# XingqunQi-lab/EmotionGestures

Hardware: AMD Instinct MI355X
Metric: gesture clips/sec (34 frames, 43 joints) (higher is better)
Workload: dtype bf16x3; 1 GPU; TED clips: 4 s 16 kHz audio -> mel(128x124) -> CVAE sample -> generator -> 34x126 pose; global_batch=64, variant=Models_spatial_memory, parallelism=clip-sharded x1, no data-path collective, launch=hipGraph replay, 4 step(s) in flight, branch_streams=False, fold_affine=False

## Files before the change

emotiongestures_amd/_lib.py:

```python
from __future__ import annotations

import ctypes as C
import os

_HERE = os.path.dirname(os.path.abspath(__file__))
LIB_PATH = os.path.join(_HERE, "libemogest_hip.so")

EG_PREC_F32, EG_PREC_BF16X3, EG_PREC_BF16 = 0, 1, 2
PRECISIONS = {"f32": EG_PREC_F32, "fp32": EG_PREC_F32, "bf16x3": EG_PREC_BF16X3, "bf16": EG_PREC_BF16}

(PACK_RAW, PACK_LINEAR, PACK_VEC_PAD, PACK_CONV3X3, PACK_BN_SCALE, PACK_BN_SHIFT, PACK_CONV1X1, PACK_STEM,
 PACK_WN_TAP, PACK_CONV1D, PACK_POS_TABLE, PACK_LINEAR_T, PACK_LINEAR_FOLD, PACK_BIAS_FOLD, PACK_CONV1X1_BF16, PACK_WN_TAPS) = range(16)


class EgError(RuntimeError):
    pass


class EgWeightEntry(C.Structure):
    _fields_ = [("key", C.c_char * 192), ("kind", C.c_int32), ("dims", C.c_int32 * 4),
                ("offset", C.c_int64), ("numel", C.c_int64)]


class EgGeneratorConfig(C.Structure):
# ... 82 lines not shown
    "eg_resample_stream_reset": (C.c_int, [_P, _I, _I, _I, _P, _P]),
    "eg_resample_stream_push": (C.c_int, [_P, _I, _I, _I, _P, _P, _I, _P, _P, _I, _P]),
    "eg_skeleton_check": (C.c_int, [_P, _P, _P, _I]),
    "eg_skeleton_out_frames": (_L, [_L, _I, _I]),
    "eg_skeleton_tile_frames": (_I, []),
    "eg_skeleton_joints": (C.c_int, [_P, _I, _I, _P, _P, _P, _I, _P, _P, _I, _I, _P, _I, _I, _I, _P, _L, _P]),
    "eg_skeleton_dir_vec": (C.c_int, [_P, _I, _I, _P, _P, _P, _I, _P, _P, _I, _I, _P, _P, _P]),
    "eg_skeleton_rest_check": (C.c_int, [_P, _I]),
    "eg_skeleton_levels": (C.c_int, [_P, _P, _P, _I, _P, _P]),
    "eg_skeleton_rotations": (C.c_int, [_P, _I, _I, _P, _P, _P, _I, _P, _P, _P, _I, _I, _P, _I, _I, _I, _P, _L, _P]),
    "eg_beat_tables": (C.c_int, [_P, _P, _P, _P]),
    "eg_beat_workspace_bytes": (_L, [_I, _I]),
    "eg_beat_align": (C.c_int, [_P, _I, _I, _P, _I, _I, _I, _I, _I, C.c_double, _I, _P, _P, _P, _P, _P, _L, _P, _P, _P, _P, _P, _P, _P]),
    "eg_beat_tracks_meta_ints": (_L, [_I]),
    "eg_beat_tracks_meta": (C.c_int, [_P, _P, _P, _I, _I, _P]),
    "eg_beat_tracks_workspace_bytes": (_L, [_P, _P, _I, _I, _I]),
    "eg_beat_align_tracks": (C.c_int, [_P, _I, _L, _P, _P, _P, _I, _I, _I, _P, _I, _I, _P, C.c_double, _I, _P, _P, _P, _P, _P, _L, _P, _P, _P,
                                       _P, _P, _P, _P]),
    "eg_beat_tracks_scan": (C.c_int, [_P, _P, _I, _P, _P, _L, _P, _P, _P]),
    "eg_take_meta_ints": (_L, [_I]),
    "eg_take_meta": (C.c_int, [_P, _I, _P]),
    "eg_track_rows_pack": (C.c_int, [_P, _I, _I, _I, _I, _P, _P, _P, _P]),
    "eg_take_distance_workspace_bytes": (_L, [_P, _I, _I]),
    "eg_take_distance": (C.c_int, [_P, _I, _I, _I, _P, _P, _I, _P, _L, _P, _P, _P]),
    "eg_conv3x3": (C.c_int, [_P, _P, _P, _P, _P, _P, _P, _I, _I, _I, _I, _I, _I, _I, _I, _I, _P]),
    "eg_conv3x3_se": (C.c_int, [_P, _P, _P, _P, _P, _P, _P, _P, _P, _I, _I, _I, _I, _I, _I, _I, _I, _I, _P]),
    "eg_se_gate_pre": (C.c_int, [_P, _P, _I, _P, _P, _P, _P, _P, _P, _P, _P, _I, _I, _I, _I, _P]),
    "eg_se_block_fused": (C.c_int, [_P] * 19 + [_I] * 7 + [_P]),
    "eg_conv3x3_gap_tiles": (_I, [_I, _I, _I, _I, _I]),
    "eg_conv3x3_channel_split": (_I, [_I, _I, _I, _I, _I, _I, _I]),
    "eg_stem_conv": (C.c_int, [_P, _P, _P, _P, _P, _P, _I, _I, _I, _I, _P]),
    "eg_se_gate": (C.c_int, [_P, _I, _P, _P, _P, _P, _P, _I, _I, _I, _P]),
    "eg_se_residual_relu": (C.c_int, [_P, _P, _P, _P, _P, _P, _P, _I, _I, _I, _I, _I, _I, _I, _I, _P]),
    "eg_linear": (C.c_int, [_P, _I, _P, _I, _P, _P, _P, _I, _P, _I, _I, _I, _I, _I, _I, _I, _I, _P]),
    "eg_split_tiles": (C.c_int, [_P, _I, _I, _I, _P, _P]),
    "eg_linear_presplit": (C.c_int, [_P, _I, _P, _I, _P, _P, _P, _I, _P, _I, _I, _I, _I, _I, _I, _P]),
    "eg_linear_presplit_causal": (C.c_int, [_P, _I, _P, _P, _I, _P, _P, _I, _P, _I, _P, _I, _I, _I, _I, _I, _I, _I, _I, _P]),
    "eg_linear_splitk": (C.c_int, [_P, _I, _P, _I, _P, _P, _I, _I, _I, _I, _I, _I, _P, _I, _P]),
    "eg_layernorm": (C.c_int, [_P, _P, _P, _P, _I, _I, C.c_float, _P]),
    "eg_attention": (C.c_int, [_P, _I, _P, _I, _P, _I, _P, _I, _P, _I, _I, _I, _I, _I, _I, _P]),
    "eg_attention_masked": (C.c_int, [_P, _I, _P, _I, _P, _I, _P, _L, _I, _P, _I, _P, _I, _I, _I, _I, _I, _I, _P]),
    "eg_mha_workspace_bytes": (_L, [_I, _I, _I, _I, _I]),
    "eg_multi_head_attention": (C.c_int, [_P, _P, _P, _P, _P, _P, _P, _P, _P, _P, _I, _I, _I, _I, _I, _I, _P, _L, _P]),
    "eg_ffn_workspace_bytes": (_L, [_I, _I, _I]),
    "eg_positionwise_ffn": (C.c_int, [_P, _P, _P, _P, _P, _P, _P, _P, _I, _I, _I, _I, _P, _L, _P]),
    "eg_tcn_forward": (C.c_int, [_P, _P, _P, _I, _I, _I, _I, _I, _P, _L, _P]),
    "eg_add_rows": (C.c_int, [_P, _P, _P, _L, _I, _I, _P]),
    "eg_add_rows_split": (C.c_int, [_P, _P, _P, _P, _L, _I, _I, _P]),
    "eg_conv3x3_packed_floats": (_L, [_I, _I]),
    "eg_profile_enable": (C.c_int, [_I]),
    "eg_profile_disable": (C.c_int, []),
    "eg_profile_read": (_I, [_P, _P, _P, _I]),
    "eg_profile_read_workgroups": (_I, [_P, _I]),
    "eg_reparameterize": (C.c_int, [_P, _P, _P, _P, _L, _P]),
    "eg_conv1d": (C.c_int, [_P, _P, _P, _P, _P, _P, _I, _I, _I, _I, _I, _I, _I, _I, _P]),
    "eg_contrastive_workspace_bytes": (C.c_int64, [_I]),
    "eg_contrastive_loss": (C.c_int, [_P, _P, _I, _I, _P, _P, _P, _P, _L, _P]),
    "eg_contrastive_backward_workspace_bytes": (_L, [_I]),
    "eg_contrastive_loss_backward": (C.c_int, [_P, _P, _I, _I, _P, _P, _P, _L, _P]),
    "eg_transpose": (C.c_int, [_P, _I, _I, _I, _P, _I, _P]),
    "eg_gemm_tn_workspace_floats": (_L, [_I, _I, _L]),
    "eg_gemm_tn": (C.c_int, [_P, _I, _P, _I, _P, _I, _I, _I, _L, _P, _L, _I, _P]),
    "eg_conv3x3_wgrad": (C.c_int, [_P, _P, _P, _I, _I, _I, _I, _I, _I, _P, _L, _P]),
    "eg_im2col3x3": (C.c_int, [_P, _P, _I, _I, _I, _I, _I, _I, _P]),
    "eg_subsample": (C.c_int, [_P, _P, _I, _I, _I, _I, _I, _I, _P]),
    "eg_conv1d_cl_forward": (C.c_int, [_P, _P, _P, _P] + [_I] * 9 + [_P]),
    "eg_conv1d_cl_backward_input": (C.c_int, [_P, _P, _P, _P] + [_I] * 9 + [_P]),
    "eg_conv1d_cl_backward_weight_workspace_floats": (_L, [_I] * 7),
    "eg_conv1d_cl_backward_weight": (C.c_int, [_P, _P, _P, _P, _P] + [_I] * 9 + [_P, _L, _P]),
    "eg_pad_cols": (C.c_int, [_P, _P, _L, _I, _I, _P]),
    "eg_colreduce_workspace_floats": (_L, [_I]),
    "eg_bn_train_forward": (C.c_int, [_P, _P, _P, _P, _P, _P, _P, _P, _L, _I, C.c_float, C.c_float, _P, _P]),
    "eg_bn_train_backward": (C.c_int, [_P, _P, _P, _P, _P, _P, _P, _P, _L, _I, _I, _P, _P]),
    "eg_bn_train_forward_gap": (C.c_int, [_P, _P, _I, _I, _P, _P, _P, _P, _P, _P, _P, _P, _L, _I, C.c_float, C.c_float, _P, _P]),
    "eg_bn_train_forward_sq": (C.c_int, [_P, _P, _P, _I, _I, _P, _P, _P, _P, _P, _P, _P, _P, _L, _I, C.c_float, C.c_float, _P, _P]),
    "eg_conv3x3_sq": (C.c_int, [_P, _P, _P, _P, _P, _P] + [_I] * 8 + [_P]),
    "eg_se_gate_train_forward": (C.c_int, [_P] * 12 + [_I, _I, _I, _P]),
    "eg_se_tail_forward": (C.c_int, [_P] * 9 + [_I, _I, _I, _P]),
    "eg_se_tail_backward_reduce": (C.c_int, [_P] * 7 + [_I, _I, _I, _P, _P]),
    "eg_se_gate_train_backward": (C.c_int, [_P] * 16 + [_I, _I, _I, _P]),
    "eg_se_tail_backward_finish": (C.c_int, [_P] * 14 + [_I, _I, _I, _P]),
    "eg_se_tail_backward_apply": (C.c_int, [_P] * 13 + [_I, _I, _I, _P]),
    "eg_colsum": (C.c_int, [_P, _P, _P, _P, _L, _I, _P, _P]),
    "eg_elementwise": (C.c_int, [_P, _P, _P, _L, _I, C.c_float, _P]),
    "eg_conv3x3_wgrad_mfma_workspace_floats": (_L, [_I, _I, _I, _I, _I]),
    "eg_conv3x3_wgrad_mfma": (C.c_int, [_P, _P, _P, _I, _I, _I, _I, _I, _P, _L, _P]),
    "eg_conv3x3_wgrad_mfma_oihw": (C.c_int, [_P, _P, _P, _I, _I, _I, _I, _I, _P, _L, _P]),
    "eg_conv3x3_wgrad_gather_mfma": (C.c_int, [_P, _P, _P, _I, _I, _I, _I, _I, _I, _P, _L, _P]),
    "eg_conv3x3_dgrad_s2": (C.c_int, [_P, _P, _P, _P, _I, _I, _I, _I, _I, _I, _P]),
    "eg_conv3x3_res_masked": (C.c_int, [_P, _P, _P, _P, _P, _I, _I, _I, _I, _I, _I, _P]),
    "eg_conv3x3_wgrad_mfma_oihw_in_affine": (C.c_int, [_P, _P, _P, _P, _P, _I, _I, _I, _I, _I, _P, _L, _P]),
    "eg_conv3x3_sq_in_affine": (C.c_int, [_P, _P, _P, _P, _P, _P, _P, _P, _I, _I, _I, _I, _I, _I, _I, _I, _P]),
    "eg_bn_train_stats_sq": (C.c_int, [_P, _P, _I, _I, _P, _P, _P, _P, _P, _P, _P, _P, _L, _I, C.c_float, C.c_float, _P, _P]),
    "eg_pack_conv3x3_device": (C.c_int, [_P, _I, _I, _I, _P, _P]),
    "eg_linear_packed_floats": (_L, [_I, _I]),
    "eg_pack_linear_device": (C.c_int, [_P, _I, _I, _I, _I, _P, _P]),
    "eg_pack_table_blocks": (_I, [_I, _I, _I, _I]),
    "eg_pack_table": (C.c_int, [_P, _I, _I, _P]),
    "eg_dropout": (C.c_int, [_P, _P, _L, C.c_float, C.c_uint32, C.c_uint64, _P]),
    "eg_dropout_dev": (C.c_int, [_P, _P, _L, C.c_float, C.c_uint32, C.c_uint64, _P, _P]),
    "eg_seg_mean": (C.c_int, [_P, _P, _I, _I, _I, C.c_float, _P, _P]),
    "eg_seg_dot": (C.c_int, [_P, _P, _P, _I, _I, _I, _P, _P]),
    "eg_se_scale": (C.c_int, [_P, _P, _P, _P, _I, _I, _I, _P]),
    "eg_layernorm_backward": (C.c_int, [_P, _P, _P, _P, _P, _I, _I, C.c_float, _P]),
    "eg_attention_train": (C.c_int, [_P, _I, _P, _I, _P, _I, _P, _I, _P, _I, _I, _I, _I, _I, C.c_float, C.c_uint32, C.c_uint64, _P, _P]),
    "eg_attention_backward_train": (C.c_int, [_P, _I, _P, _I, _P, _I, _P, _P, _I, _P, _I, _P, _I, _P, _I, _I, _I, _I, _I, _I, C.c_float, C.c_uint32,
# ... 57 lines not shown
```

emotiongestures_amd/csrc/mel.hip:

```cpp
#include "common.h"
#include "beat_shared.h"
#include <hip/hip_fp16.h>
#include <math.h>

namespace {

__global__ __launch_bounds__(256) void mel_power_kernel(const float* __restrict__ audio, int n_samples, const float* __restrict__ melfb_t,
                                                        const float* __restrict__ window, const float* __restrict__ twiddle,
                                                        const int* __restrict__ band, float* __restrict__ melpow, int n_frames) {
    __shared__ float re[1024], im[1024];
    const int f0 = blockIdx.x * 2, f1 = f0 + 1, b = blockIdx.y, tid = threadIdx.x;
    const float* clip = audio + (size_t)b * n_samples;
    for (int i = tid; i < 1024; i += 256) {
        const int s0 = f0 * 512 - 512 + i, s1 = s0 + 512;
        const float wv = window[i];
        const int r = (int)(__brev((unsigned)i) >> 22);
        re[r] = (s0 >= 0 && s0 < n_samples) ? clip[s0] * wv : 0.f;
        im[r] = (f1 < n_frames && s1 >= 0 && s1 < n_samples) ? clip[s1] * wv : 0.f;
    }
    __syncthreads();
#pragma unroll 1
    for (int s = 0; s < 10; ++s) {
        const int half = 1 << s;
#pragma unroll
        for (int u = 0; u < 2; ++u) {
            const int j = tid + u * 256;
            const int pos = j & (half - 1), i0 = ((j >> s) << (s + 1)) + pos, i1 = i0 + half;
            const int tw = pos << (9 - s);
            const float c = twiddle[2 * tw], sn = twiddle[2 * tw + 1];
            const float xr = re[i1], xi = im[i1];
            const float tr = xr * c - xi * sn, ti = xr * sn + xi * c;
            const float ar = re[i0], ai = im[i0];
            re[i0] = ar + tr; im[i0] = ai + ti;
            re[i1] = ar - tr; im[i1] = ai - ti;
        }
        __syncthreads();
    }
    float pa[3], pb[3];
#pragma unroll
    for (int u = 0; u < 3; ++u) {
        const int k = u < 2 ? tid + u * 256 : 512, nk = (1024 - k) & 1023;
        pa[u] = pb[u] = 0.f;
        if (u < 2 || tid == 0) {
            const float zr = re[k], zi = im[k], yr = re[nk], yi = im[nk];
            const float r0 = 0.5f * (zr + yr), i0 = 0.5f * (zi - yi);
            const float r1 = 0.5f * (zi + yi), i1 = 0.5f * (yr - zr);
            pa[u] = r0 * r0 + i0 * i0;
            pb[u] = r1 * r1 + i1 * i1;
        }
    }
    __syncthreads();
    re[tid] = pa[0]; re[tid + 256] = pa[1];
    im[tid] = pb[0]; im[tid + 256] = pb[1];
    if (tid == 0) { re[512] = pa[2]; im[512] = pb[2]; }
    __syncthreads();
    const int m = tid & 127, fr = tid >> 7, f = f0 + fr;
    const float* pw = fr ? im : re;
    const int b0 = band[2 * m], b1 = band[2 * m + 1];
    float s = 0.f;
    for (int k = b0; k < b1; ++k) s += melfb_t[k * 128 + m] * pw[k];
    if (f < n_frames) melpow[((size_t)b * 128 + m) * n_frames + f] = s;
}

__global__ __launch_bounds__(1024) void mel_db_kernel(const float* __restrict__ melpow, float* __restrict__ spec, int n_frames,
                                                      int out_frames) {
    __shared__ float red[16];
    const int b = blockIdx.x, tid = threadIdx.x;
    const float* p = melpow + (size_t)b * 128 * n_frames;
    float mx = 0.f;
    for (int i = tid; i < 128 * n_frames; i += 1024) mx = fmaxf(mx, p[i]);
    mx = wave_max(mx);
    if ((tid & 63) == 0) red[tid >> 6] = mx;
    __syncthreads();
    mx = red[0];
#pragma unroll
    for (int w = 1; w < 16; ++w) mx = fmaxf(mx, red[w]);
    const float inv_ref = 1.0f / fmaxf(1e-10f, mx);
    const float floor_db = -80.f;
    for (int i = tid; i < 128 * out_frames; i += 1024) {
        const int m = i / out_frames, f = i - m * out_frames;
        float db = 10.f * log10f(fmaxf(1e-10f, p[m * n_frames + f]) * inv_ref);
        db = fmaxf(db, floor_db);
        spec[((size_t)b * 128 + m) * out_frames + f] = __half2float(__float2half_rn(db));
    }
}

double hz_to_mel(double f) {
    const double f_sp = 200.0 / 3, min_log_hz = 1000.0, min_log_mel = min_log_hz / f_sp, logstep = log(6.4) / 27.0;
    return f >= min_log_hz ? min_log_mel + log(f / min_log_hz) / logstep : f / f_sp;
}
double mel_to_hz(double m) {
    const double f_sp = 200.0 / 3, min_log_hz = 1000.0, min_log_mel = min_log_hz / f_sp, logstep = log(6.4) / 27.0;
    return m >= min_log_mel ? min_log_hz * exp(logstep * (m - min_log_mel)) : f_sp * m;
}

}

namespace {

void mel_tables_host(int n_fft, float* h_melfb_t, float* h_window, float* h_twiddle, int32_t* h_band) {
    const int n_mels = 128, n_bins = n_fft / 2 + 1;
    const double sr = 16000.0;
    double hz[130];
    const double m_lo = hz_to_mel(0.0), m_hi = hz_to_mel(sr / 2);
    for (int i = 0; i < n_mels + 2; ++i) hz[i] = mel_to_hz(m_lo + (m_hi - m_lo) * i / (n_mels + 1));
    for (int m = 0; m < n_mels; ++m) {
        const double enorm = 2.0 / (hz[m + 2] - hz[m]);
        for (int k = 0; k < n_bins; ++k) {
            const double fk = (sr / 2) * k / (n_bins - 1);
            const double lower = (fk - hz[m]) / (hz[m + 1] - hz[m]);
            const double upper = (hz[m + 2] - fk) / (hz[m + 2] - hz[m + 1]);
            double w = lower < upper ? lower : upper;
            if (w < 0) w = 0;
            h_melfb_t[k * 128 + m] = (float)(w * enorm);
        }
        int lo = n_bins, hi = 0;
        for (int k = 0; k < n_bins; ++k)
            if (h_melfb_t[k * 128 + m] != 0.f) { if (k < lo) lo = k; hi = k + 1; }
        if (lo > hi) lo = hi = 0;
        h_band[2 * m] = lo; h_band[2 * m + 1] = hi;
    }
    const double pi = 3.14159265358979323846;
    for (int i = 0; i < n_fft; ++i) h_window[i] = (float)(0.5 - 0.5 * cos(2.0 * pi * i / n_fft));
    for (int t = 0; t < n_fft / 2; ++t) {
        h_twiddle[2 * t] = (float)cos(2.0 * pi * t / n_fft);
        h_twiddle[2 * t + 1] = (float)(-sin(2.0 * pi * t / n_fft));
    }
}

}

extern "C" int eg_mel_tables(float* h_melfb_t, float* h_window, float* h_twiddle, int32_t* h_band) {
    EG_REQUIRE(h_melfb_t && h_window && h_twiddle && h_band, EG_ERR_BAD_ARG, "eg_mel_tables: null pointer");
    mel_tables_host(1024, h_melfb_t, h_window, h_twiddle, h_band);
    return EG_OK;
}

extern "C" int64_t eg_mel_workspace_bytes(int32_t batch, int32_t n_samples) {
    const int n_frames = 1 + n_samples / 512;
    return (int64_t)batch * 128 * n_frames * (int64_t)sizeof(float);
}

extern "C" int eg_melspectrogram(const float* audio, int32_t batch, int32_t n_samples, const float* d_melfb_t,
                                 const float* d_window, const float* d_twiddle, const int32_t* d_band, float* spec, int32_t out_frames,
                                 void* workspace, int64_t workspace_bytes, void* stream) {
    EG_REQUIRE(audio && d_melfb_t && d_window && d_twiddle && d_band && spec && workspace, EG_ERR_BAD_ARG, "eg_melspectrogram: null pointer");
    EG_REQUIRE(batch > 0 && n_samples >= 512, EG_ERR_BAD_ARG, "eg_melspectrogram: batch=%d n_samples=%d", batch, n_samples);
    const int n_frames = 1 + n_samples / 512;
    EG_REQUIRE(out_frames > 0 && out_frames <= n_frames, EG_ERR_BAD_ARG, "eg_melspectrogram: out_frames=%d of %d", out_frames, n_frames);
    EG_REQUIRE(workspace_bytes >= eg_mel_workspace_bytes(batch, n_samples), EG_ERR_WORKSPACE, "eg_melspectrogram: workspace too small");
    hipStream_t st = (hipStream_t)stream;
    float* melpow = reinterpret_cast<float*>(workspace);
    hipLaunchKernelGGL(mel_power_kernel, dim3((n_frames + 1) / 2, batch), dim3(256), 0, st, audio, n_samples, d_melfb_t, d_window, d_twiddle,
                       d_band, melpow, n_frames);
    int rc = eg_check_launch("mel_power");
    if (rc) return rc;
    hipLaunchKernelGGL(mel_db_kernel, dim3(batch), dim3(1024), 0, st, melpow, spec, n_frames, out_frames);
    return eg_check_launch("mel_db");
}

#define EG_BEAT_MAX_EVENTS (EG_BEAT_MAX_FRAMES / 2 + 1)

namespace {

__global__ __launch_bounds__(256) void beat_stft_kernel(const float* __restrict__ audio, int n_samples, const float* __restrict__ melfb_t,
                                                        const float* __restrict__ window, const float* __restrict__ twiddle,
                                                        const int* __restrict__ band, float* __restrict__ meldb, float* __restrict__ rms,
                                                        int n_frames) {
    const int b = blockIdx.y;
    beat_stft_frames(audio + (size_t)b * n_samples, n_samples, melfb_t, window, twiddle, band, meldb + (size_t)b * 128 * n_frames,
                     rms + (size_t)b * n_frames, n_frames, blockIdx.x * 2);
}

__device__ double gahr(const short* __restrict__ ev, int n_ev, const short* __restrict__ pb, int n_pb, int fps, double sigma) {
    return beat_gahr(ev, n_ev, pb, n_pb, fps, sigma);
}

__global__ __launch_bounds__(256) void beat_align_kernel(const float* __restrict__ meldb, const float* __restrict__ rms_ws, int n_frames,
                                                         const float* __restrict__ pose, int pose_frames, int pose_dim, int fps, int r_lo,
                                                         int r_hi, double sigma, int order, double* __restrict__ score,
                                                         int* __restrict__ n_audio_beats, float* __restrict__ oenv_out,
                                                         float* __restrict__ rms_out, uint8_t* __restrict__ audio_mask,
                                                         uint8_t* __restrict__ pose_mask) {
    __shared__ float oenv[EG_BEAT_MAX_FRAMES], x[EG_BEAT_MAX_FRAMES], rms[EG_BEAT_MAX_FRAMES];
    __shared__ uint8_t fl[3][EG_BEAT_MAX_FRAMES];
    uint8_t* cand = fl[0];
    uint8_t* min_o = fl[1];
    uint8_t* min_r = fl[2];
    __shared__ short ev[3][EG_BEAT_MAX_EVENTS];
    __shared__ float vel[8][EG_BEAT_MAX_FRAMES];
    __shared__ short pbeat[8][EG_BEAT_MAX_EVENTS];
    __shared__ int n_pb[8];
    __shared__ float redf[2][4];
    __shared__ int n_ev_s, any_s;
    __shared__ double g24[24];
    const int b = blockIdx.x, tid = threadIdx.x, T = n_frames;
    const float* db = meldb + (size_t)b * 128 * T;

    float mx = -INFINITY;
    for (int i = tid; i < 128 * T; i += 256) mx = fmaxf(mx, db[i]);
    mx = wave_max(mx);
    if ((tid & 63) == 0) redf[0][tid >> 6] = mx;
    __syncthreads();
    const float floor_db = fmaxf(fmaxf(redf[0][0], redf[0][1]), fmaxf(redf[0][2], redf[0][3])) - 80.f;
    for (int t = tid; t < T; t += 256) {
        float s = 0.f;
        if (t >= 3)
// ... 173 lines not shown
```

emotiongestures_amd/csrc/misc.hip:

```cpp
#include "common.h"

namespace {

template <int NV>
__global__ __launch_bounds__(256) void layernorm_kernel(const float* __restrict__ x, const float* __restrict__ g,
                                                        const float* __restrict__ b, float* __restrict__ y, int rows, int D,
                                                        float eps, unsigned short* __restrict__ img) {
    const int row = blockIdx.x * 4 + (threadIdx.x >> 6), lane = threadIdx.x & 63;
    if (row >= rows) return;
    const f4* xr = reinterpret_cast<const f4*>(x + (size_t)row * D);
    const int nq = D >> 2;
    f4 v[NV];
    float s = 0.f;
#pragma unroll
    for (int i = 0; i < NV; ++i) {
        const int q = lane + i * 64;
        v[i] = q < nq ? xr[q] : (f4){0.f, 0.f, 0.f, 0.f};
        s += (v[i][0] + v[i][1]) + (v[i][2] + v[i][3]);
    }
    const float m0 = wave_sum(s) / (float)D;
    float c = 0.f;
#pragma unroll
    for (int i = 0; i < NV; ++i) {
        const int q = lane + i * 64;
        if (q < nq) {
            const f4 d = v[i] - m0;
            c += (d[0] + d[1]) + (d[2] + d[3]);
        }
    }
    const float mean = m0 + wave_sum(c) / (float)D;
    float ss = 0.f;
#pragma unroll
    for (int i = 0; i < NV; ++i) {
        const int q = lane + i * 64;
        if (q < nq) {
            const f4 d = v[i] - mean;
            ss += (d[0] * d[0] + d[1] * d[1]) + (d[2] * d[2] + d[3] * d[3]);
        }
    }
    const float rstd = 1.0f / sqrtf(wave_sum(ss) / (float)D + eps);
    f4* yr = reinterpret_cast<f4*>(y + (size_t)row * D);
#pragma unroll
    for (int i = 0; i < NV; ++i) {
        const int q = lane + i * 64;
        if (q < nq) {
            const f4 o = (v[i] - mean) * rstd * reinterpret_cast<const f4*>(g)[q] + reinterpret_cast<const f4*>(b)[q];
            yr[q] = o;
            if (img) {
                const f4 z = (f4){0.f, 0.f, 0.f, 0.f};
                bf8 h8, l8;
                split_octet<true>(o, z, h8, l8);
                const int KO = D >> 3;
                const size_t slot = (((size_t)(row >> 6) * KO + (q >> 1)) * 64 + (row & 63)) * 8 + (q & 1) * 4;
// ... 51 lines not shown
    const size_t total = (size_t)((rows + 63) >> 6) * 64 * KO;
    for (size_t i = (size_t)blockIdx.x * 256 + threadIdx.x; i < total; i += (size_t)gridDim.x * 256) {
        if (zero && i < (size_t)64 * KO) zero[i] = (bf8){0, 0, 0, 0, 0, 0, 0, 0};
        const int t = (int)(i / (64 * KO)), rem = (int)(i - (size_t)t * 64 * KO), o = rem >> 6, r = t * 64 + (rem & 63), k = o * 8;
        if (r >= rows) continue;
        int64_t w = idx[r];
        w = w < 0 ? 0 : (w >= n_words ? n_words - 1 : w);
        f4 v0 = (f4){0.f, 0.f, 0.f, 0.f}, v1 = v0;
        if (k < dim) v0 = *reinterpret_cast<const f4*>(table + (size_t)w * dim + k);
        if (k + 4 < dim) v1 = *reinterpret_cast<const f4*>(table + (size_t)w * dim + k + 4);
        *reinterpret_cast<f4*>(out + (size_t)r * ld + k) = v0;
        *reinterpret_cast<f4*>(out + (size_t)r * ld + k + 4) = v1;
        bf8 h, l;
        split_octet<true>(v0, v1, h, l);
        const size_t slot = ((size_t)(r >> 6) * KO + o) * 64 + (r & 63);
        hi[slot] = h;
        lo[slot] = l;
    }
}

__global__ __launch_bounds__(256) void add_kernel(const f4* __restrict__ a, const f4* __restrict__ b, f4* __restrict__ out,
                                                  size_t n4, int row_q, int period) {
    for (size_t i = (size_t)blockIdx.x * 256 + threadIdx.x; i < n4; i += (size_t)gridDim.x * 256) {
        size_t j = i;
        if (period) {
            const size_t row = i / row_q;
            j = (row % period) * row_q + (i - row * row_q);
        }
        out[i] = a[i] + b[j];
    }
}

__global__ __launch_bounds__(256) void add_img_kernel(const f4* __restrict__ a, const f4* __restrict__ b, f4* __restrict__ out, bf8* __restrict__ hi,
                                                      bf8* __restrict__ lo, size_t rows, int row_o, int period) {
    const size_t total = ((rows + 63) >> 6) * 64 * row_o;
    for (size_t t = (size_t)blockIdx.x * 256 + threadIdx.x; t < total; t += (size_t)gridDim.x * 256) {
        const size_t tile = t / (64 * (size_t)row_o);
        const int rem = (int)(t - tile * 64 * row_o), o = rem >> 6;
        const size_t row = tile * 64 + (rem & 63);
        if (row >= rows) continue;
        const size_t i = row * row_o + o;
        const size_t j = period ? (row % period) * row_o + o : i;
        const f4 v0 = a[2 * i] + b[2 * j], v1 = a[2 * i + 1] + b[2 * j + 1];
        out[2 * i] = v0;
        out[2 * i + 1] = v1;
        bf8 h, l;
        split_octet<true>(v0, v1, h, l);
        const size_t slot = ((row >> 6) * row_o + o) * 64 + (row & 63);
        hi[slot] = h;
        lo[slot] = l;
    }
}

__global__ __launch_bounds__(256) void time_linear_kernel(const float* __restrict__ x, const float* __restrict__ w,
                                                          const float* __restrict__ bias, float* __restrict__ y, int L, int C, int ld) {
    extern __shared__ __attribute__((aligned(16))) float sm[];
    float* Ws = sm;
    float* Xs = sm + L * L;
    const int b = blockIdx.y, c0 = blockIdx.x * 64, tid = threadIdx.x;
    for (int i = tid; i < L * L; i += 256) Ws[i] = w[i];
    for (int i = tid; i < L * 64; i += 256) {
        const int t = i >> 6, c = i & 63;
        Xs[i] = (c0 + c < C) ? x[((size_t)b * L + t) * ld + c0 + c] : 0.f;
    }
    __syncthreads();
    const int c = tid & 63;
    if (c0 + c >= C) return;
    for (int tp = tid >> 6; tp < L; tp += 4) {
        float s = bias[tp];
        for (int t = 0; t < L; ++t) s += Ws[tp * L + t] * Xs[t * 64 + c];
        y[((size_t)b * L + tp) * ld + c0 + c] = s;
    }
}

struct PriorArgs {
    const float* prior;
    const float *w1, *b1, *s1, *t1;
    const float *w2, *b2, *s2, *t2;
    const float *sp_w0, *sp_b0, *sp_w1, *sp_b1;
    const float *tc_w0, *tc_b0, *tc_w1, *tc_b1;
    const float *tm_w0, *tm_b0, *tm_w1, *tm_b1;
    float* cat;
    float* tm_mem;
    float* tm_pe;
    int P, PL, D, Dpad, chunk, variant, stage_w, dchunk;
};

__device__ __forceinline__ float block_dot(const float* __restrict__ wrow, const float* __restrict__ xs, int n, int lane) {
    float s = 0.f;
    for (int i = lane; i < n; i += 64) s += wrow[i] * xs[i];
    return wave_sum(s);
}

__global__ __launch_bounds__(256) void prior_pred_kernel(PriorArgs a) {
    extern __shared__ __attribute__((aligned(16))) float sm[];
    const int b = blockIdx.x, tid = threadIdx.x, wave = tid >> 6, lane = tid & 63;
    const int P = a.P, PL = a.PL, D = a.D;
    const int d0 = blockIdx.y * a.dchunk, dc = min(a.dchunk, D - d0);
    const int XW = dc + 4, HW = dc + 2;
    float* xs = sm;
    float* h1 = xs + P * XW;
    float* h2 = h1 + PL * HW;
    float* v0 = h2 + PL * dc;
    float* v1 = v0 + (a.variant == 1 ? a.chunk * D : 0);
    float* v2 = v1 + (a.variant == 1 ? D : 0);
    float* w1s = v2 + (a.variant == 1 ? D : 0);
    float* w2s = w1s + PL * P * 3;
    if (a.stage_w) {
        for (int i = tid; i < PL * P * 3; i += 256) w1s[i] = a.w1[i];
        for (int i = tid; i < PL * PL * 3; i += 256) w2s[i] = a.w2[i];
    }
    const float* w1p = a.stage_w ? w1s : a.w1;
    const float* w2p = a.stage_w ? w2s : a.w2;
    for (int i = tid; i < P * XW; i += 256) {
        const int f = i / XW, d = d0 - 2 + (i - f * XW);
        xs[i] = (d >= 0 && d < D) ? a.prior[((size_t)b * P + f) * D + d] : 0.f;
    }
    __syncthreads();
    for (int i = tid; i < PL * HW; i += 256) {
        const int co = i / HW, j = i - co * HW, d = d0 - 1 + j;
        float v = 0.f;
        if (d >= 0 && d < D) {
            float s = a.b1[co];
            for (int ci = 0; ci < P; ++ci) {
                const float* wp = w1p + (co * P + ci) * 3;
// ... 529 lines not shown
    EG_REQUIRE(a && table && out && images && rows > 0 && d > 0 && (d & 63) == 0, EG_ERR_BAD_ARG, "eg_add_rows_split: null pointer, empty shape or d %% 64 != 0");
    return egi_add_img(a, table, out, images, (size_t)rows * d, d, period, (hipStream_t)stream);
}

extern "C" int eg_window_gather(const float* audio, int32_t utterances, int64_t total_samples, int32_t windows, int64_t hop_samples,
                                int32_t n_samples, float* out, void* stream) {
    EG_REQUIRE(audio && out, EG_ERR_BAD_ARG, "eg_window_gather: null pointer");
    EG_REQUIRE(utterances >= 1 && windows >= 1, EG_ERR_BAD_ARG, "eg_window_gather: utterances=%d windows=%d", utterances, windows);
    EG_REQUIRE(total_samples >= 1 && hop_samples >= 1 && n_samples >= 1, EG_ERR_BAD_ARG, "eg_window_gather: total_samples=%lld hop_samples=%lld n_samples=%d",
               (long long)total_samples, (long long)hop_samples, n_samples);
    EG_REQUIRE((int64_t)(windows - 1) * hop_samples < total_samples, EG_ERR_BAD_ARG,
               "eg_window_gather: windows=%d: the last window starts at sample %lld of %lld", windows, (long long)(windows - 1) * hop_samples,
               (long long)total_samples);
    hipLaunchKernelGGL(window_gather_kernel, dim3(grid_for((size_t)utterances * windows * n_samples)), dim3(256), 0, (hipStream_t)stream, audio, out,
                       utterances, total_samples, windows, hop_samples, n_samples);
    return eg_check_launch("window_gather");
}

int egi_embedding(const int64_t* idx, const float* table, float* out, int rows, int dim, int ld, int n_words, hipStream_t st) {
    hipLaunchKernelGGL(embedding_kernel, dim3(grid_for((size_t)rows * dim / 4)), dim3(256), 0, st, idx, table, out, rows, dim, ld, n_words);
    return eg_check_launch("embedding");
}
int egi_add(const float* a, const float* b, float* out, size_t n, int row_len, int period, hipStream_t st);
int egi_embedding_img(const int64_t* idx, const float* table, float* out, void* img, void* zero_line, int rows, int dim, int ld, int n_words, hipStream_t st) {
    EG_REQUIRE((dim & 3) == 0 && (ld & 63) == 0 && ld >= dim, EG_ERR_ALIGN, "embedding: dim %% 4, ld %% 64");
    bf8* hi = reinterpret_cast<bf8*>(img);
    bf8* lo = hi + (size_t)eg_cdiv(rows, 64) * (ld >> 3) * 64;
    hipLaunchKernelGGL(embedding_img_kernel, dim3(grid_for((size_t)eg_cdiv(rows, 64) * 64 * (ld >> 3))), dim3(256), 0, st, idx, table, out, hi, lo,
                       reinterpret_cast<bf8*>(zero_line), rows, dim, ld, n_words);
    return eg_check_launch("embedding");
}
int egi_add_img(const float* a, const float* b, float* out, void* img, size_t n, int row_len, int period, hipStream_t st) {
    if (!img) return egi_add(a, b, out, n, row_len, period, st);
    EG_REQUIRE((row_len & 63) == 0, EG_ERR_ALIGN, "add: image output needs row_len %% 64 == 0");
    const size_t rows = n / row_len;
    bf8* hi = reinterpret_cast<bf8*>(img);
    bf8* lo = hi + ((rows + 63) >> 6) * (size_t)(row_len >> 3) * 64;
    hipLaunchKernelGGL(add_img_kernel, dim3(grid_for(n / 8)), dim3(256), 0, st, reinterpret_cast<const f4*>(a), reinterpret_cast<const f4*>(b),
                       reinterpret_cast<f4*>(out), hi, lo, rows, row_len / 8, period);
    return eg_check_launch("add");
}
int egi_add(const float* a, const float* b, float* out, size_t n, int row_len, int period, hipStream_t st) {
    hipLaunchKernelGGL(add_kernel, dim3(grid_for(n / 4)), dim3(256), 0, st, reinterpret_cast<const f4*>(a),
                       reinterpret_cast<const f4*>(b), reinterpret_cast<f4*>(out), n / 4, row_len / 4, period);
    return eg_check_launch("add");
}
int egi_add_bcast(const float* a, const float* b, float* out, size_t rows, int row_len, int period, int rep, hipStream_t st) {
    const size_t n4 = rows * (size_t)(row_len / 4);
    hipLaunchKernelGGL(add_bcast_kernel, dim3(grid_for(n4)), dim3(256), 0, st, reinterpret_cast<const f4*>(a),
                       reinterpret_cast<const f4*>(b), reinterpret_cast<f4*>(out), n4, row_len / 4, period, rep);
    return eg_check_launch("add_bcast");
}
int egi_time_linear(const float* x, const float* w, const float* bias, float* y, int batch, int L, int C, int ld, hipStream_t st) {
    const size_t smem = sizeof(float) * ((size_t)L * L + (size_t)L * 64);
    hipLaunchKernelGGL(time_linear_kernel, dim3(eg_cdiv(C, 64), batch), dim3(256), smem, st, x, w, bias, y, L, C, ld);
    return eg_check_launch("time_linear");
}
int egi_copy2d(const float* src, int lds_, float* dst, int ldd, int rows, int cols, hipStream_t st) {
    hipLaunchKernelGGL(copy2d_kernel, dim3(grid_for((size_t)rows * cols)), dim3(256), 0, st, src, lds_, dst, ldd, rows, cols);
    return eg_check_launch("copy2d");
}

int egi_swap01(const void* in, void* out, int A, int B, size_t inner_words, hipStream_t st) {
    if ((inner_words & 3) == 0 && eg_aligned16(in) && eg_aligned16(out)) {
        const size_t q = inner_words / 4;
        hipLaunchKernelGGL((swap01_kernel<u32x4_t>), dim3(grid_for((size_t)A * B * q)), dim3(256), 0, st, reinterpret_cast<const u32x4_t*>(in),
                           reinterpret_cast<u32x4_t*>(out), A, B, q);
    } else {
        hipLaunchKernelGGL((swap01_kernel<unsigned int>), dim3(grid_for((size_t)A * B * inner_words)), dim3(256), 0, st,
                           reinterpret_cast<const unsigned int*>(in), reinterpret_cast<unsigned int*>(out), A, B, inner_words);
    }
    return eg_check_launch("swap01");
}
int egi_rollout_handoff(const float* pose, const float* prior_in, const float* alpha, float* track, float* windows, float* prior_out, int U,
                        int W, int w, int F, int P, int D, hipStream_t st) {
    hipLaunchKernelGGL(rollout_handoff_kernel, dim3(grid_for((size_t)U * F * D)), dim3(256), 0, st, pose, prior_in, alpha, track, windows,
                       prior_out, U, W, w, F, P, D);
    return eg_check_launch("rollout_handoff");
}

struct EgiPriorW {
    const float *w1, *b1, *s1, *t1, *w2, *b2, *s2, *t2;
    const float *sp_w0, *sp_b0, *sp_w1, *sp_b1, *tc_w0, *tc_b0, *tc_w1, *tc_b1, *tm_w0, *tm_b0, *tm_w1, *tm_b1;
};
int egi_prior_encoder(const float* prior, const EgiPriorW& w, float* cat, float* tm_mem, float* tm_pe, float* tm_gram,
                      int batch, int P, int F, int D, int Dpad, int chunk, int variant, hipStream_t st) {
    PriorArgs a;
    a.prior = prior; a.w1 = w.w1; a.b1 = w.b1; a.s1 = w.s1; a.t1 = w.t1; a.w2 = w.w2; a.b2 = w.b2; a.s2 = w.s2; a.t2 = w.t2;
    a.sp_w0 = w.sp_w0; a.sp_b0 = w.sp_b0; a.sp_w1 = w.sp_w1; a.sp_b1 = w.sp_b1;
    a.tc_w0 = w.tc_w0; a.tc_b0 = w.tc_b0; a.tc_w1 = w.tc_w1; a.tc_b1 = w.tc_b1;
    a.tm_w0 = w.tm_w0; a.tm_b0 = w.tm_b0; a.tm_w1 = w.tm_w1; a.tm_b1 = w.tm_b1;
    a.cat = cat; a.tm_mem = tm_mem; a.tm_pe = tm_pe;
    a.P = P; a.PL = F - P; a.D = D; a.Dpad = Dpad; a.chunk = chunk; a.variant = variant;
    const int PL = F - P;
    a.dchunk = variant == 1 ? D : (D < 64 ? D : 64);
    const int dc = a.dchunk;
    const size_t base = sizeof(float) * ((size_t)P * (dc + 4) + (size_t)PL * (dc + 2) + (size_t)PL * dc +
                                         (variant == 1 ? (size_t)chunk * D + 2 * (size_t)D : 0));
    const size_t wbytes = sizeof(float) * ((size_t)PL * P * 3 + (size_t)PL * PL * 3);
    a.stage_w = (base + wbytes <= 160 * 1024) ? 1 : 0;
    const size_t smem = base + (a.stage_w ? wbytes : 0);
    if (smem > 160 * 1024) { eg_set_error("prior encoder: LDS need %zu B", smem); return EG_ERR_UNSUPPORTED; }
    if (int rc = eg_ensure_dynamic_lds(reinterpret_cast<const void*>(prior_pred_kernel), smem, "prior encoder")) return rc;
    hipLaunchKernelGGL(prior_pred_kernel, dim3(batch, eg_cdiv(D, dc)), dim3(256), smem, st, a);
    int rc = eg_check_launch("prior_pred");
    if (rc || variant != 1) return rc;
    hipLaunchKernelGGL(tm_gram_kernel, dim3(eg_cdiv(D * chunk, 256)), dim3(256), 0, st, tm_mem, tm_pe, tm_gram, batch, D, chunk);
    if ((rc = eg_check_launch("tm_gram"))) return rc;
    hipLaunchKernelGGL(tm_apply_kernel, dim3(batch), dim3(64), 0, st, tm_mem, tm_gram, cat, D, Dpad, chunk, P, F);
// ... 275 lines not shown
```

include/emogest.h:

```cpp
#ifndef EMOGEST_H
#define EMOGEST_H

#include <stddef.h>
#include <stdint.h>

#ifdef __cplusplus
extern "C" {
#endif

typedef enum EgStatus {
    EG_OK = 0,
    EG_ERR_BAD_ARG = -1,
    EG_ERR_UNSUPPORTED = -2,
    EG_ERR_WORKSPACE = -3,
    EG_ERR_HIP = -4,
    EG_ERR_ALIGN = -5
} EgStatus;

typedef enum EgPrecision {
    EG_PREC_F32 = 0,
    EG_PREC_BF16X3 = 1,
    EG_PREC_BF16 = 2
} EgPrecision;

// ... 273 lines not shown
                       int32_t m, int32_t n, int32_t k, int32_t relu, int32_t precision, void* stream);
int eg_linear_presplit_causal(const void* x_images, int32_t k_x, const void* zero_line, const float* w, int32_t ldw, const float* bias,
                              const float* res2, int32_t ldr, float* y, int32_t ldc, void* y_images, int32_t y_k, int32_t m, int32_t n,
                              int32_t k_tap, int32_t relu, int32_t shift, int32_t period, int32_t precision, void* stream);

int eg_linear_splitk(const float* x, int32_t lda, const float* w, int32_t ldw, const float* bias, float* y,
                     int32_t ldc, int32_t m, int32_t n, int32_t k, int32_t relu, int32_t splits,
                     float* partial, int32_t precision, void* stream);

typedef struct EgLinearArgs {
    const float* x; const float* w; const float* bias; const float* res1; const float* res2; float* y;
    const float* gate_src;
    const int32_t* drop_epoch;
    float* partial;
    const void* x_images;
    void* y_images;
    uint64_t drop_offset;
    int32_t lda, ldw, ldr, ldc, ldg;
    int32_t m, n, k, relu, precision, splits;
    int32_t k_x, y_k;
    uint32_t drop_seed;
    float drop_p;
} EgLinearArgs;
int eg_linear_ex(const EgLinearArgs* args, void* stream);

int eg_layernorm(const float* x, const float* gamma, const float* beta, float* y, int32_t rows, int32_t d,
                 float eps, void* stream);
int eg_layernorm_img(const float* x, const float* gamma, const float* beta, float* y, void* y_images, int32_t rows, int32_t d, float eps,
                     void* stream);

int eg_attention(const float* q, int32_t ldq, const float* k, int32_t ldk, const float* v, int32_t ldv,
                 float* out, int32_t ldo, float* attn, int32_t batch, int32_t heads, int32_t lq, int32_t lk,
                 int32_t dk, int32_t precision, void* stream);
int eg_attention_masked(const float* q, int32_t ldq, const float* k, int32_t ldk, const float* v, int32_t ldv, const uint8_t* mask,
                        int64_t mask_batch_stride, int32_t mask_query_stride, float* out, int32_t ldo, float* attn, int32_t batch,
                        int32_t heads, int32_t lq, int32_t lk, int32_t dk, int32_t precision, void* stream);

int64_t eg_mha_workspace_bytes(int32_t batch, int32_t lq, int32_t lk, int32_t d_model, int32_t heads);
int eg_multi_head_attention(const float* xq, const float* xkv, const float* wq, const float* wk, const float* wv,
                            const float* wo, const float* ln_g, const float* ln_b, float* out, float* attn,
                            int32_t batch, int32_t lq, int32_t lk, int32_t d_model, int32_t heads,
                            int32_t precision, void* workspace, int64_t workspace_bytes, void* stream);

int64_t eg_ffn_workspace_bytes(int32_t rows, int32_t d_model, int32_t d_inner);
int eg_positionwise_ffn(const float* x, const float* w1, const float* b1, const float* w2, const float* b2,
                        const float* ln_g, const float* ln_b, float* out, int32_t rows, int32_t d_model,
                        int32_t d_inner, int32_t precision, void* workspace, int64_t workspace_bytes, void* stream);

int eg_tcn_forward(const float* x, const float* w, float* y, int32_t batch, int32_t len, int32_t c,
                   int32_t levels, int32_t precision, void* workspace, int64_t workspace_bytes, void* stream);

int eg_add_rows_split(const float* a, const float* table, float* out, void* images, int64_t rows, int32_t d, int32_t period, void* stream);
int eg_add_rows(const float* a, const float* table, float* out, int64_t rows, int32_t d, int32_t period, void* stream);

int eg_reparameterize(const float* mu, const float* logvar, const float* eps, float* z, int64_t n, void* stream);

int eg_conv1d(const float* x, const float* w, const float* bias, const float* scale, const float* shift, float* y, int32_t n,
              int32_t cin, int32_t cout, int32_t lin, int32_t k, int32_t stride, int32_t pad, int32_t act, void* stream);

int64_t eg_contrastive_workspace_bytes(int32_t n);
int eg_contrastive_loss(const float* face, const float* audio, int32_t n, int32_t d, float* cross, float* loss, float* acc,
                        void* workspace, int64_t workspace_bytes, void* stream);
int64_t eg_contrastive_backward_workspace_bytes(int32_t n);
int eg_contrastive_loss_backward(const float* face, const float* audio, int32_t n, int32_t d, float* gface, float* gaudio, void* workspace,
                                 int64_t workspace_bytes, void* stream);



int eg_transpose(const float* x, int32_t ldx, int32_t rows, int32_t cols, float* y, int32_t ldy, void* stream);
int64_t eg_gemm_tn_workspace_floats(int32_t m, int32_t n, int64_t k);
int eg_gemm_tn(const float* a, int32_t lda, const float* b, int32_t ldb, float* c, int32_t ldc, int32_t m, int32_t n, int64_t k,
               float* workspace, int64_t workspace_floats, int32_t accumulate, void* stream);
int eg_conv3x3_wgrad(const float* x, const float* dy, float* dw_mat, int32_t batch, int32_t h, int32_t w, int32_t cin, int32_t cout,
                     int32_t stride, float* workspace, int64_t workspace_floats, void* stream);
int eg_im2col3x3(const float* x, float* col, int32_t batch, int32_t h, int32_t w, int32_t c, int32_t stride, int32_t backward, void* stream);
int eg_subsample(const float* x, float* y, int32_t batch, int32_t h, int32_t w, int32_t c, int32_t stride, int32_t backward, void* stream);
int eg_conv1d_cl_forward(const float* x, const float* w, const float* bias, float* y, int32_t batch, int32_t len, int32_t cin, int32_t len_out,
                         int32_t cout, int32_t k, int32_t stride, int32_t pad, int32_t dilation, void* stream);
int eg_conv1d_cl_backward_input(const float* dy, const float* w, const float* bias, float* dx, int32_t batch, int32_t len, int32_t cin,
                                int32_t len_out, int32_t cout, int32_t k, int32_t stride, int32_t pad, int32_t dilation, void* stream);
int64_t eg_conv1d_cl_backward_weight_workspace_floats(int32_t batch, int32_t cin, int32_t len_out, int32_t cout, int32_t k, int32_t stride,
                                                      int32_t dilation);
int eg_conv1d_cl_backward_weight(const float* x, const float* dy, float* dw, float* db_dy, float* db_x, int32_t batch, int32_t len, int32_t cin,
                                 int32_t len_out, int32_t cout, int32_t k, int32_t stride, int32_t pad, int32_t dilation, float* workspace,
                                 int64_t workspace_floats, void* stream);
int eg_pad_cols(const float* x, float* y, int64_t rows, int32_t k, int32_t k_padded, void* stream);
int64_t eg_colreduce_workspace_floats(int32_t c);
int eg_bn_train_forward(const float* x, const float* gamma, const float* beta, float* y, float* save_mean, float* save_rstd,
                        float* running_mean, float* running_var, int64_t rows, int32_t c, float momentum, float eps, float* workspace,
                        void* stream);
int eg_bn_train_backward(const float* x, const float* dy, const float* gamma, const float* save_mean, const float* save_rstd, float* dx,
                         float* dgamma, float* dbeta, int64_t rows, int32_t c, int32_t relu_mask, float* workspace, void* stream);
int eg_bn_train_forward_gap(const float* x, const float* gap_partial, int32_t tiles, int32_t batch, const float* gamma, const float* beta,
                            float* y, float* save_mean, float* save_rstd, float* clip_sum, float* running_mean, float* running_var,
                            int64_t rows, int32_t c, float momentum, float eps, float* workspace, void* stream);
int eg_bn_train_forward_sq(const float* x, const float* gap_partial, const float* gap_sq_partial, int32_t tiles, int32_t batch, const float* gamma,
                           const float* beta, float* y, float* save_mean, float* save_rstd, float* clip_sum, float* running_mean, float* running_var,
                           int64_t rows, int32_t c, float momentum, float eps, float* workspace, void* stream);
int eg_bn_train_stats_sq(const float* gap_partial, const float* gap_sq_partial, int32_t tiles, int32_t batch, const float* gamma, const float* beta,
                         float* save_mean, float* save_rstd, float* running_mean, float* running_var, float* aff_scale, float* aff_shift, int64_t rows,
                         int32_t c, float momentum, float eps, float* workspace, void* stream);
int eg_se_gate_train_forward(const float* clip_sum, const float* mean, const float* rstd, const float* gamma, const float* beta, const float* w1,
                             const float* b1, const float* w2, const float* b2, float* pooled, float* h, float* gate, int32_t batch, int32_t hw,
                             int32_t c, void* stream);
int eg_se_tail_forward(const float* c2, const float* res, const float* mean, const float* rstd, const float* gamma, const float* beta,
                       const float* gate, float* out, uint32_t* relu_bits, int32_t batch, int32_t hw, int32_t c, void* stream);
// ... 74 lines not shown
```

Baseline: 27040 clips/s.

## Use radix-4 mel FFT and register-blocked time-linear kernel

Replaces the radix-2 shared-memory FFT in the mel power kernel with a five-pass radix-4 FFT. It keeps values in registers between passes, uses swizzled LDS slots and twiddles staged in LDS, and unrolls the mel filterbank dot product by eight. Rewrites the time-linear kernel so each thread accumulates several output rows in registers, reading padded weights as float4 and staging loads in batches. The old kernels stay selectable through environment variables, and a public eg_time_linear entry point is added. The extra getenv calls add host cost per launch, though hipGraph replay hides that.

```diff
diff --git a/emotiongestures_amd/_lib.py b/emotiongestures_amd/_lib.py
--- a/emotiongestures_amd/_lib.py
+++ b/emotiongestures_amd/_lib.py
@@ -158,6 +158,7 @@
     "eg_profile_disable": (C.c_int, []),
     "eg_profile_read": (_I, [_P, _P, _P, _I]),
     "eg_profile_read_workgroups": (_I, [_P, _I]),
+    "eg_time_linear": (C.c_int, [_P, _P, _P, _P, _I, _I, _I, _I, _P]),
     "eg_reparameterize": (C.c_int, [_P, _P, _P, _P, _L, _P]),
     "eg_conv1d": (C.c_int, [_P, _P, _P, _P, _P, _P, _I, _I, _I, _I, _I, _I, _I, _I, _P]),
     "eg_contrastive_workspace_bytes": (C.c_int64, [_I]),
diff --git a/emotiongestures_amd/csrc/mel.hip b/emotiongestures_amd/csrc/mel.hip
--- a/emotiongestures_amd/csrc/mel.hip
+++ b/emotiongestures_amd/csrc/mel.hip
@@ -2,12 +2,14 @@
 #include "beat_shared.h"
 #include <hip/hip_fp16.h>
 #include <math.h>
+#include <stdlib.h>
+#include <string.h>
 
 namespace {
 
-__global__ __launch_bounds__(256) void mel_power_kernel(const float* __restrict__ audio, int n_samples, const float* __restrict__ melfb_t,
-                                                        const float* __restrict__ window, const float* __restrict__ twiddle,
-                                                        const int* __restrict__ band, float* __restrict__ melpow, int n_frames) {
+__global__ __launch_bounds__(256) void mel_power_radix2_kernel(const float* __restrict__ audio, int n_samples, const float* __restrict__ melfb_t,
+                                                               const float* __restrict__ window, const float* __restrict__ twiddle,
+                                                               const int* __restrict__ band, float* __restrict__ melpow, int n_frames) {
     __shared__ float re[1024], im[1024];
     const int f0 = blockIdx.x * 2, f1 = f0 + 1, b = blockIdx.y, tid = threadIdx.x;
     const float* clip = audio + (size_t)b * n_samples;
@@ -59,6 +61,120 @@
     const int b0 = band[2 * m], b1 = band[2 * m + 1];
     float s = 0.f;
     for (int k = b0; k < b1; ++k) s += melfb_t[k * 128 + m] * pw[k];
+    if (f < n_frames) melpow[((size_t)b * 128 + m) * n_frames + f] = s;
+}
+
+__device__ __forceinline__ int fft_slot(int i) { return i ^ (5 * ((i >> 4) & 3)); }
+
+__device__ __forceinline__ float2 cmul(float2 a, float2 b) { return make_float2(a.x * b.x - a.y * b.y, a.x * b.y + a.y * b.x); }
+
+__device__ __forceinline__ int tw_slot(int t) { return t + (t >> 4); }
+template <int NS>
+__device__ __forceinline__ void fft_twiddles(const float2* tw, int j, float2 (&w)[3]) {
+    const int t = (j & (NS - 1)) * (256 / NS), t3 = 3 * t;
+    w[0] = tw[tw_slot(t)];
+    w[1] = tw[tw_slot(2 * t)];
+    const float2 x = tw[tw_slot(t3 & 511)];
+    w[2] = t3 < 512 ? x : make_float2(-x.x, -x.y);
+}
+
+template <int NS>
+__device__ __forceinline__ void fft_pass(float2 (&v)[4], const float2 (&w)[3], float2* __restrict__ out, int j) {
+    if (NS > 1) {
+#pragma unroll
+        for (int r = 1; r < 4; ++r) v[r] = cmul(v[r], w[r - 1]);
+    }
+    const float2 a0 = make_float2(v[0].x + v[2].x, v[0].y + v[2].y), a1 = make_float2(v[0].x - v[2].x, v[0].y - v[2].y);
+    const float2 a2 = make_float2(v[1].x + v[3].x, v[1].y + v[3].y), a3 = make_float2(v[1].y - v[3].y, v[3].x - v[1].x);
+    const int k = j & (NS - 1), base = ((j - k) << 2) + k;
+    out[fft_slot(base)] = make_float2(a0.x + a2.x, a0.y + a2.y);
+    out[fft_slot(base + NS)] = make_float2(a1.x + a3.x, a1.y + a3.y);
+    out[fft_slot(base + 2 * NS)] = make_float2(a0.x - a2.x, a0.y - a2.y);
+    out[fft_slot(base + 3 * NS)] = make_float2(a1.x - a3.x, a1.y - a3.y);
+}
+
+__device__ __forceinline__ void fft_gather(float2 (&v)[4], const float2* __restrict__ in, int j) {
+#pragma unroll
+    for (int r = 0; r < 4; ++r) v[r] = in[fft_slot(j + 256 * r)];
+}
+
+__global__ __launch_bounds__(256) void mel_power_kernel(const float* __restrict__ audio, int n_samples, const float* __restrict__ melfb_t,
+                                                        const float* __restrict__ window, const float* __restrict__ twiddle,
+                                                        const int* __restrict__ band, float* __restrict__ melpow, int n_frames) {
+    __shared__ float2 za[1024], zb[1024];
+    const int f0 = blockIdx.x * 2, f1 = f0 + 1, b = blockIdx.y, tid = threadIdx.x;
+    const float* clip = audio + (size_t)b * n_samples;
+    float raw[6];
+    const int s0 = f0 * 512 - 512 + tid;
+#pragma unroll
+    for (int u = 0; u < 6; ++u) {
+        const int s = s0 + 256 * u;
+        raw[u] = (s >= 0 && s < n_samples) ? clip[s] : 0.f;
+    }
+    float2 v[4];
+#pragma unroll
+    for (int q = 0; q < 4; ++q) {
+        const float wv = window[tid + 256 * q];
+        v[q] = make_float2(raw[q] * wv, f1 < n_frames ? raw[q + 2] * wv : 0.f);
+    }
+    {
+        const float2* tw = reinterpret_cast<const float2*>(twiddle);
+        const float2 ta = tw[tid], tb = tw[tid + 256];
+        zb[tw_slot(tid)] = ta;
+        zb[tw_slot(tid + 256)] = tb;
+    }
+    const int m = tid >> 1, fr = tid & 1, f = f0 + fr;
+    const int b0 = band[2 * m], b1 = band[2 * m + 1];
+    __syncthreads();
+    float2 w1[3], w2[3], w3[3], w4[3];
+    fft_twiddles<4>(zb, tid, w1);
+    fft_twiddles<16>(zb, tid, w2);
+    fft_twiddles<64>(zb, tid, w3);
+    fft_twiddles<256>(zb, tid, w4);
+    float2 none[3];
+    fft_pass<1>(v, none, za, tid);
+    __syncthreads();
+    fft_gather(v, za, tid);
+    fft_pass<4>(v, w1, zb, tid);
+    __syncthreads();
+    fft_gather(v, zb, tid);
+    fft_pass<16>(v, w2, za, tid);
+    __syncthreads();
+    fft_gather(v, za, tid);
+    fft_pass<64>(v, w3, zb, tid);
+    __syncthreads();
+    fft_gather(v, zb, tid);
+    fft_pass<256>(v, w4, za, tid);
+    __syncthreads();
+    float pa[3], pb[3];
+#pragma unroll
+    for (int u = 0; u < 3; ++u) {
+        const int k = u < 2 ? tid + u * 256 : 512, nk = (1024 - k) & 1023;
+        pa[u] = pb[u] = 0.f;
+        if (u < 2 || tid == 0) {
+            const float2 z = za[fft_slot(k)], y = za[fft_slot(nk)];
+            const float r0 = 0.5f * (z.x + y.x), i0 = 0.5f * (z.y - y.y);
+            const float r1 = 0.5f * (z.y + y.y), i1 = 0.5f * (y.x - z.x);
+            pa[u] = r0 * r0 + i0 * i0;
+            pb[u] = r1 * r1 + i1 * i1;
+        }
+    }
+    float* re = reinterpret_cast<float*>(zb);
+    float* im = re + 1024;
+    re[tid] = pa[0]; re[tid + 256] = pa[1];
+    im[tid] = pb[0]; im[tid + 256] = pb[1];
+    if (tid == 0) { re[512] = pa[2]; im[512] = pb[2]; }
+    __syncthreads();
+    const float* pw = fr ? im : re;
+    float s = 0.f;
+    for (int k0 = b0; k0 < b1; k0 += 8) {
+        float wv[8];
+#pragma unroll
+        for (int u = 0; u < 8; ++u) wv[u] = k0 + u < b1 ? melfb_t[(k0 + u) * 128 + m] : 0.f;
+#pragma unroll
+        for (int u = 0; u < 8; ++u)
+            if (k0 + u < b1) s += wv[u] * pw[k0 + u];
+    }
     if (f < n_frames) melpow[((size_t)b * 128 + m) * n_frames + f] = s;
 }
 
@@ -149,10 +265,17 @@
     const int n_frames = 1 + n_samples / 512;
     EG_REQUIRE(out_frames > 0 && out_frames <= n_frames, EG_ERR_BAD_ARG, "eg_melspectrogram: out_frames=%d of %d", out_frames, n_frames);
     EG_REQUIRE(workspace_bytes >= eg_mel_workspace_bytes(batch, n_samples), EG_ERR_WORKSPACE, "eg_melspectrogram: workspace too small");
+    const char* fft = getenv("EG_MEL_FFT");
+    const bool radix2 = fft && !strcmp(fft, "2");
+    EG_REQUIRE(!fft || !fft[0] || radix2 || !strcmp(fft, "4"), EG_ERR_BAD_ARG, "EG_MEL_FFT=\"%s\": accepted values are \"4\" and \"2\" (unset or empty: 4)", fft);
     hipStream_t st = (hipStream_t)stream;
     float* melpow = reinterpret_cast<float*>(workspace);
-    hipLaunchKernelGGL(mel_power_kernel, dim3((n_frames + 1) / 2, batch), dim3(256), 0, st, audio, n_samples, d_melfb_t, d_window, d_twiddle,
-                       d_band, melpow, n_frames);
+    if (radix2)
+        hipLaunchKernelGGL(mel_power_radix2_kernel, dim3((n_frames + 1) / 2, batch), dim3(256), 0, st, audio, n_samples, d_melfb_t, d_window,
+                           d_twiddle, d_band, melpow, n_frames);
+    else
+        hipLaunchKernelGGL(mel_power_kernel, dim3((n_frames + 1) / 2, batch), dim3(256), 0, st, audio, n_samples, d_melfb_t, d_window, d_twiddle,
+                           d_band, melpow, n_frames);
     int rc = eg_check_launch("mel_power");
     if (rc) return rc;
     hipLaunchKernelGGL(mel_db_kernel, dim3(batch), dim3(1024), 0, st, melpow, spec, n_frames, out_frames);
diff --git a/emotiongestures_amd/csrc/misc.hip b/emotiongestures_amd/csrc/misc.hip
--- a/emotiongestures_amd/csrc/misc.hip
+++ b/emotiongestures_amd/csrc/misc.hip
@@ -1,4 +1,6 @@
 #include "common.h"
+#include <stdlib.h>
+#include <string.h>
 
 namespace {
 
@@ -156,7 +158,7 @@
     }
 }
 
-__global__ __launch_bounds__(256) void time_linear_kernel(const float* __restrict__ x, const float* __restrict__ w,
+__global__ __launch_bounds__(256) void time_linear_ref_kernel(const float* __restrict__ x, const float* __restrict__ w,
                                                           const float* __restrict__ bias, float* __restrict__ y, int L, int C, int ld) {
     extern __shared__ __attribute__((aligned(16))) float sm[];
     float* Ws = sm;
@@ -175,6 +177,79 @@
         for (int t = 0; t < L; ++t) s += Ws[tp * L + t] * Xs[t * 64 + c];
         y[((size_t)b * L + tp) * ld + c0 + c] = s;
     }
+}
+
+template <int R>
+__device__ __forceinline__ void time_linear_rows(const float* Ws, const float* Xs, const float* __restrict__ bias, float* __restrict__ yc, int tp0,
+                                                 int L, int Lp, int ld, int c) {
+    float acc[R];
+#pragma unroll
+    for (int k = 0; k < R; ++k) acc[k] = bias[tp0 + 4 * k];
+    const float* wr = Ws + tp0 * Lp;
+    const int L4 = L & ~3;
+    int t = 0;
+#pragma unroll 2
+    for (; t < L4; t += 4) {
+        float xv[4];
+#pragma unroll
+        for (int u = 0; u < 4; ++u) xv[u] = Xs[(t + u) * 64 + c];
+#pragma unroll
+        for (int k = 0; k < R; ++k) {
+            const f4 wv = *reinterpret_cast<const f4*>(wr + 4 * k * Lp + t);
+            acc[k] += wv.x * xv[0];
+            acc[k] += wv.y * xv[1];
+            acc[k] += wv.z * xv[2];
+            acc[k] += wv.w * xv[3];
+        }
+    }
+    for (; t < L; ++t) {
+        const float xv = Xs[t * 64 + c];
+#pragma unroll
+        for (int k = 0; k < R; ++k) acc[k] += wr[4 * k * Lp + t] * xv;
+    }
+#pragma unroll
+    for (int k = 0; k < R; ++k) yc[(size_t)(tp0 + 4 * k) * ld] = acc[k];
+}
+
+__global__ __launch_bounds__(256) void time_linear_kernel(const float* __restrict__ x, const float* __restrict__ w,
+                                                          const float* __restrict__ bias, float* __restrict__ y, int L, int C, int ld) {
+    extern __shared__ __attribute__((aligned(16))) float sm[];
+    const int Lp = (L + 3) & ~3;
+    float* Ws = sm;
+    float* Xs = sm + L * Lp;
+    const int b = blockIdx.y, c0 = blockIdx.x * 64, tid = threadIdx.x, c = tid & 63;
+    const bool live = c0 + c < C;
+    const float* xc = x + (size_t)b * L * ld + c0 + c;
+    for (int i0 = tid; i0 < L * max(L, 64); i0 += 16 * 256) {
+        float vx[16], vw[16];
+#pragma unroll
+        for (int u = 0; u < 16; ++u) {
+            const int i = i0 + u * 256;
+            vx[u] = (live && i < L * 64) ? xc[(size_t)(i >> 6) * ld] : 0.f;
+        }
+#pragma unroll
+        for (int u = 0; u < 16; ++u) {
+            const int i = i0 + u * 256;
+            vw[u] = i < L * L ? w[i] : 0.f;
+        }
+#pragma unroll
+        for (int u = 0; u < 16; ++u) {
+            const int i = i0 + u * 256;
+            if (i < L * 64) Xs[i] = vx[u];
+        }
+#pragma unroll
+        for (int u = 0; u < 16; ++u) {
+            const int i = i0 + u * 256, r = i / L;
+            if (i < L * L) Ws[r * Lp + (i - r * L)] = vw[u];
+        }
+    }
+    __syncthreads();
+    int tp = __builtin_amdgcn_readfirstlane(tid >> 6);
+    if (!live) return;
+    float* yc = y + (size_t)b * L * ld + c0 + c;
+    for (; tp + 56 < L; tp += 60) time_linear_rows<15>(Ws, Xs, bias, yc, tp, L, Lp, ld, c);
+    for (; tp + 16 < L; tp += 20) time_linear_rows<5>(Ws, Xs, bias, yc, tp, L, Lp, ld, c);
+    for (; tp < L; tp += 4) time_linear_rows<1>(Ws, Xs, bias, yc, tp, L, Lp, ld, c);
 }
 
 struct PriorArgs {
@@ -810,9 +885,22 @@
     return eg_check_launch("add_bcast");
 }
 int egi_time_linear(const float* x, const float* w, const float* bias, float* y, int batch, int L, int C, int ld, hipStream_t st) {
-    const size_t smem = sizeof(float) * ((size_t)L * L + (size_t)L * 64);
-    hipLaunchKernelGGL(time_linear_kernel, dim3(eg_cdiv(C, 64), batch), dim3(256), smem, st, x, w, bias, y, L, C, ld);
+    const char* e = getenv("EG_TIME_LINEAR");
+    const bool ref = e && !strcmp(e, "ref");
+    EG_REQUIRE(!e || !e[0] || ref, EG_ERR_BAD_ARG, "EG_TIME_LINEAR=\"%s\": the only accepted value is \"ref\" (unset or empty: register-blocked)", e);
+    const size_t smem = sizeof(float) * ((size_t)L * (ref ? L : (L + 3) & ~3) + (size_t)L * 64);
+    EG_REQUIRE(smem <= 65536, EG_ERR_UNSUPPORTED, "time_linear: L=%d needs %zu bytes of LDS", L, smem);
+    if (ref)
+        hipLaunchKernelGGL(time_linear_ref_kernel, dim3(eg_cdiv(C, 64), batch), dim3(256), smem, st, x, w, bias, y, L, C, ld);
+    else
+        hipLaunchKernelGGL(time_linear_kernel, dim3(eg_cdiv(C, 64), batch), dim3(256), smem, st, x, w, bias, y, L, C, ld);
     return eg_check_launch("time_linear");
+}
+extern "C" int eg_time_linear(const float* x, const float* w, const float* bias, float* y, int32_t batch, int32_t len, int32_t c, int32_t ld,
+                              void* stream) {
+    EG_REQUIRE(x && w && bias && y, EG_ERR_BAD_ARG, "eg_time_linear: null pointer");
+    EG_REQUIRE(batch > 0 && len > 0 && c > 0 && ld >= c, EG_ERR_BAD_ARG, "eg_time_linear: batch=%d len=%d c=%d ld=%d", batch, len, c, ld);
+    return egi_time_linear(x, w, bias, y, batch, len, c, ld, (hipStream_t)stream);
 }
 int egi_copy2d(const float* src, int lds_, float* dst, int ldd, int rows, int cols, hipStream_t st) {
     hipLaunchKernelGGL(copy2d_kernel, dim3(grid_for((size_t)rows * cols)), dim3(256), 0, st, src, lds_, dst, ldd, rows, cols);
diff --git a/include/emogest.h b/include/emogest.h
--- a/include/emogest.h
+++ b/include/emogest.h
@@ -349,6 +349,8 @@
 
 int eg_add_rows_split(const float* a, const float* table, float* out, void* images, int64_t rows, int32_t d, int32_t period, void* stream);
 int eg_add_rows(const float* a, const float* table, float* out, int64_t rows, int32_t d, int32_t period, void* stream);
+
+int eg_time_linear(const float* x, const float* w, const float* bias, float* y, int32_t batch, int32_t len, int32_t c, int32_t ld, void* stream);
 
 int eg_reparameterize(const float* mu, const float* logvar, const float* eps, float* z, int64_t n, void* stream);
 
```

After: 27470 clips/s, median of 6. 1.6% higher.
